# Findeton/mpi-vision

Hardware: AMD Instinct MI355X
Metric: rendered Mpix/sec (node) + achieved HBM GB/s fraction, 1024²×128-plane MPI (higher is better)
Workload: dtype f32

## Files before the change

### mpi_vision_amd/csrc/abi.hip

```cpp
#include <cstdio>
#include <cstdarg>
#include <cstring>
#include <cstdlib>
#include <algorithm>
#include <mutex>
#include <type_traits>

#include "../../include/mpiv.h"

#ifndef MPIV_AB
#define MPIV_AB 0
#endif
#include "render.hip"
#include "render_lds.hip"
#include "render_chunk.hip"
#include "render_ring.hip"
#include "render_mv.hip"
#include "render_bwd.hip"
#include "render_bwd_cam.hip"
#include "sweep.hip"
#include "warp_bwd.hip"
#include "psv_bwd.hip"
#include "helper_bwd.hip"
#include "geometry.hip"
#include "assemble.hip"
#include "synth.hip"
#include "render_texel.hip"

namespace {

thread_local char g_err[512] = "";

int fail(int code, const char* fmt, ...) {
    va_list ap;
    va_start(ap, fmt);
    vsnprintf(g_err, sizeof(g_err), fmt, ap);
    va_end(ap);
    return code;
}

int launched(const char* what) {
    const hipError_t e = hipGetLastError();
    if (e != hipSuccess) return fail(MPIV_ERR_HIP, "%s: launch failed: %s", what, hipGetErrorString(e));
    g_err[0] = '\0';
    return MPIV_OK;
}

inline hipStream_t S(void* s) { return reinterpret_cast<hipStream_t>(s); }
inline bool aligned16(const void* p) { return (reinterpret_cast<uintptr_t>(p) & 15) == 0; }
inline unsigned blocks(int64_t n, int per) { return (unsigned)((n + per - 1) / per); }

enum DebugOpt { kOptRenderMv, kOptRenderPair, kOptNativeLds, kOptSweepTile, kOptSweepStore, kOptBoxShrink,
                kOptRenderChunk, kOptRenderRing, kOptRenderTile, kOptBwdFallback, kOptBwdMargin, kOptSweepDlane,
                kOptRenderVshare, kOptChunkRows, kOptSweepRows, kOptChunkFlight, kOptBwdGather, kOptSweepDirect,
                kOptBwdPollLimit, kOptBwdFbBlocks, kOptBwdFbMode, kOptChunkStrip, kOptU8Flight, kOptBwdGroup,
                kOptNetoutGeo, kOptNetoutBuf, kOptBwdOverlap, kOptSweepBand, kOptSweepPf, kOptSweepSoa, kOptBwdUnfold,
                kOptNetoutFg3, kOptRenderSame, kOptRenderColsep, kOptRenderOrder, kOptChunkWide, kNumOpts };
const char* const kOptNames[kNumOpts] = {"render_mv", "render_pair", "render_native_lds",
                                         "sweep_tile", "sweep_store", "box_shrink", "render_chunk", "render_ring",
                                         "render_tile", "bwd_fallback", "bwd_margin", "sweep_dlane",
                                         "render_vshare", "chunk_rows", "sweep_rows", "chunk_flight", "bwd_gather",
                                         "sweep_direct", "bwd_poll_limit", "bwd_fb_blocks", "bwd_fb_mode",
                                         "chunk_strip", "u8_flight", "bwd_group", "netout_geo", "netout_buf", "bwd_overlap", "sweep_band",
                                         "sweep_pf", "sweep_soa", "bwd_unfold", "netout_fg3",
                                         "render_same", "render_colsep", "render_order", "chunk_wide"};
#ifndef MPIV_CHUNK_STRIP
#define MPIV_CHUNK_STRIP 1
#endif
#ifndef MPIV_U8_FLIGHT
#define MPIV_U8_FLIGHT 0
#endif
const int kOptDefaults[kNumOpts] = {0, 0, 1, 0, -1, 0, 0, 0, 0, 0, 16, 1, 0, 0, 0, 0, 0, 0, 0, 0, 0, MPIV_CHUNK_STRIP,
                                    MPIV_U8_FLIGHT, 0, 0, 1, 0, 0, 0, 0, 0, 1, 0, 0, 0, 0};
int g_opts[kNumOpts] = {0, 0, 1, 0, -1, 0, 0, 0, 0, 0, 16, 1, 0, 0, 0, 0, 0, 0, 0, 0, 0, MPIV_CHUNK_STRIP, MPIV_U8_FLIGHT, 0,
                        0, 1, 0, 0, 0, 0, 0, 1, 0, 0, 0, 0};

int opt(DebugOpt o) { return __atomic_load_n(&g_opts[o], __ATOMIC_RELAXED); }

bool ab_only(int o, int v) {
    switch (o) {
        case kOptRenderMv: case kOptRenderPair: case kOptSweepTile: return v != 0;
        case kOptRenderRing: return v > 0;
        case kOptRenderTile: return v != 0 && v != -1;
        case kOptRenderVshare: return v == -1 || v == 1;
        case kOptSweepStore: return v >= 0;
        case kOptRenderChunk: return v >= 100;
        case kOptSweepDlane: return v == 0;
        case kOptChunkRows: return v == 2 || v == 4;
        case kOptChunkFlight: return v == 4;
        case kOptChunkStrip: return v >= 2;
        case kOptSweepRows: return v == 6 || v == 8;
        case kOptBwdGather: return v == 1 || v == 2 || v == 3;
        case kOptBwdPollLimit: case kOptBwdFbBlocks: case kOptBwdFbMode: return v != 0;
        case kOptBwdOverlap: case kOptSweepBand: return v != 0;
        case kOptSweepPf: case kOptSweepSoa: return v > 0;
        default: return false;
    }
}

thread_local unsigned long long* g_census = nullptr;

struct RouteNote {
    char name[160];
    int64_t threads;
};
thread_local RouteNote* g_route = nullptr;

int note_route(int64_t blocks_, int threads, const char* fmt, ...) {
    va_list ap;
    va_start(ap, fmt);
    vsnprintf(g_route->name, sizeof(g_route->name), fmt, ap);
    va_end(ap);
    g_route->threads = blocks_ * threads;
    return MPIV_OK;
}

constexpr int64_t kMaxGridYZ = 65535;
constexpr int kNativeLdsMaxP = 16;
constexpr int kChunkMaxLds = 65536;
constexpr int kChunkSplit = 1;

constexpr int64_t kMaxGridX = 2147483647;

constexpr const char* kViewTooLarge = "%s: one view is limited to H*W < 2^26 and P*H*W < 2^31 (32 GiB of fp32 RGBA)";
inline bool view_too_large(int H, int W, int P) {
    return (int64_t)H * W >= ((int64_t)1 << 26) || (int64_t)P * H * W >= ((int64_t)1 << 31);
}

}

using namespace mpiv;

namespace {

constexpr int kOrderMinViews = 64;
int render_tile_order(int V) {
    const int o = opt(kOptRenderOrder);
    return o > 0 ? 1 : o < 0 ? 0 : V >= kOrderMinViews ? 1 : 0;
}

int chunk_rows() {
    const int o = opt(kOptChunkRows);
    return (o == 2 || o == 4) ? o : 1;
}

template <int CH, int SPLIT>
int launch_chunk(int R, const float* mpi, int64_t vstride, const RenderGeom& g, const ChunkGeom& cg, int B,
                 const float* homs, float* out, float4* ck, size_t lds, hipStream_t q, const char* nm,
                 bool wide = false) {
    if constexpr (CH == 8 && SPLIT == 1) {
        if (wide) {
            const int64_t ns = (int64_t)blocks(g.W, kStripTX) * blocks(g.H, 16) * B;
            if (ns > kMaxGridX) return fail(MPIV_ERR_ARG, "%s: too many blocks", nm);
            if (g_route) return note_route(ns, 256, "render_chunk_strip_kernel<16, 2, true>");
            render_chunk_strip_kernel<16, 2, true><<<(unsigned)ns, 256, lds, q>>>(mpi, vstride, g, cg, B, homs, out, ck);
            return launched(nm);
        }
    }
    const int64_t nb = (int64_t)blocks(g.W, kTileX) * blocks(g.H, kTileY * R) * B;
    if (nb > kMaxGridX) return fail(MPIV_ERR_ARG, "%s: too many blocks", nm);
    const int NT = (opt(kOptChunkFlight) == 4 && R == 1 && SPLIT == 1) ? 4 : 2;
    const int so = opt(kOptChunkStrip);
    if (CH == 8 && SPLIT == 1 && R == 1 && NT == 2 && so > 0) {
        const int SR = (so == 2 || so == 3) ? 8 : 16, SNT = so >= 3 ? 3 : 2;
        const int64_t ns = (int64_t)blocks(g.W, kStripTX) * blocks(g.H, SR) * B;
        if (ns > kMaxGridX) return fail(MPIV_ERR_ARG, "%s: too many blocks", nm);
        if (g_route) return note_route(ns, 256, "render_chunk_strip_kernel<%d, %d>", SR, SNT);
#if MPIV_AB
        if (so == 2)
            render_chunk_strip_kernel<8, 2><<<(unsigned)ns, 256, lds, q>>>(mpi, vstride, g, cg, B, homs, out, ck);
        else if (so == 3)
            render_chunk_strip_kernel<8, 3><<<(unsigned)ns, 256, lds, q>>>(mpi, vstride, g, cg, B, homs, out, ck);
        else if (so == 4)
// ... 261 lines not shown
    const int rows_opt = opt(kOptRenderTile);
    const int64_t rows_blocks = (int64_t)blocks(W, kTileX) * blocks(H, 4 * 8) * V;
    const bool stretched_vs = !square && rows_blocks >= 2048;
    const bool variants_off = !opt(kOptRenderMv) && !opt(kOptRenderPair);
    const int rows_auto = ((square || stretched_vs) && variants_off) ? 8 : 0;
    const int vs_opt = opt(kOptRenderVshare);
    [[maybe_unused]] const int rows_sel = fast ? (rows_opt ? rows_opt : rows_auto) : 0;
#if MPIV_AB
    if (const int rows = rows_sel; rows == 108 || rows == 116 || rows == 132) {
        const int R = rows - 100;
        const int64_t nb = (int64_t)blocks(W, kTileX) * blocks(H, 4 * R) * V;
        if (nb > kMaxGridX) return fail(MPIV_ERR_ARG, "%s: too many blocks", nm);
#define MPIV_ROWSL(R)                                                                                                  \
    if (ct)                                                                                                           \
        render_rows_lds_kernel<true, R><<<(unsigned)nb, 256, 0, st>>>(pk, ps, g, V, p_begin, p_end, back, homs, out); \
    else                                                                                                              \
        render_rows_lds_kernel<false, R><<<(unsigned)nb, 256, 0, st>>>(pk, ps, g, V, p_begin, p_end, 1, homs, out)
        if (R == 8) MPIV_ROWSL(8);
        else if (R == 16) MPIV_ROWSL(16);
        else MPIV_ROWSL(32);
#undef MPIV_ROWSL
        return launched(nm);
    }
#endif

    int vsd = 0;
    if (fast && (vs_opt == 3 || vs_opt == 4 || vs_opt == 5 || vs_opt == 11))
        vsd = vs_opt;
    else if (fast && vs_opt == 0 && !rows_opt && rows_auto == 8)
        vsd = rows_same(syr) ? 4 : V <= 2 ? 11 : V <= 8 ? 3 : square ? 4 : 5;
    if (vsd) {
        const int R = vsd == 3 ? 8 : vsd == 4 ? 6 : vsd == 5 ? 9 : 4;
        const int64_t nb = (int64_t)blocks(W, kTileX) * blocks(H, 4 * R) * V;
        if (nb > kMaxGridX) return fail(MPIV_ERR_ARG, "%s: too many blocks", nm);
        const bool same = rows_same(syr);
        const bool oob = same && vsd == 4 && rows_same_oob(V);
        if (g_route)
            return note_route(nb, 256, "render_rows_%s<%s, %d, true, false, %d, %s, %s>", tgt ? "tgt_kernel" : "kernel",
                              ct ? "true" : "false", R, vsd == 3 || vsd == 11 ? 4 : 3, same ? "true" : "false",
                              oob ? "true" : "false");
        unsigned long long* cn = (g_census && !ct) ? g_census : nullptr;
        if (cn) g_census = nullptr;
        const int csp = opt(kOptRenderColsep);
        const int ord = render_tile_order(V);
#define MPIV_VSD(R, D, SM, OB)                                                                                        \
    if (ct)                                                                                                          \
        render_rows_kernel<true, R, true, false, D, SM, OB><<<(unsigned)nb, 256, 0, st>>>(                           \
            pk, ps, g, V, p_begin, p_end, back, homs, out, nullptr, 0, -1, csp, ord);                                \
    else if (tgt)                                                                                                    \
        render_rows_tgt_kernel<false, R, true, false, D, SM, OB><<<(unsigned)nb, 256, 0, st>>>(                      \
            pk, ps, gt, V, p_begin, p_end, 1, homs, out, nullptr, 0, -1, csp, ord);                                  \
    else                                                                                                             \
        render_rows_kernel<false, R, true, false, D, SM, OB><<<(unsigned)nb, 256, 0, st>>>(                          \
            pk, ps, g, V, p_begin, p_end, 1, homs, out, nullptr, 0, -1, csp, ord)
#define MPIV_VSDC(R, D, SM, OB)                                                                                       \
    if (cn)                                                                                                          \
        render_rows_kernel<false, R, true, true, D, SM, OB><<<(unsigned)nb, 256, 0, st>>>(                           \
            pk, ps, g, V, p_begin, p_end, 1, homs, out, cn, 0, -1, csp, ord);                                        \
    else                                                                                                             \
        MPIV_VSD(R, D, SM, OB)
        if (oob) {
            MPIV_VSDC(6, 3, true, true);
        } else if (same) {
            switch (vsd) {
                case 3: MPIV_VSDC(8, 4, true, false); break;
                case 4: MPIV_VSDC(6, 3, true, false); break;
                case 5: MPIV_VSDC(9, 3, true, false); break;
                default: MPIV_VSDC(4, 4, true, false); break;
            }
        } else {
            switch (vsd) {
                case 3: MPIV_VSDC(8, 4, false, false); break;
                case 4: MPIV_VSDC(6, 3, false, false); break;
                case 5: MPIV_VSDC(9, 3, false, false); break;
                default: MPIV_VSDC(4, 4, false, false); break;
            }
        }
#undef MPIV_VSDC
#undef MPIV_VSD
        return launched(nm);
    }
#if MPIV_AB
    if (const int rows = rows_sel; rows == 2 || rows == 4 || rows == 8 || rows == 16) {
        const int64_t nb = (int64_t)blocks(W, kTileX) * blocks(H, 4 * rows) * V;
        if (nb > kMaxGridX) return fail(MPIV_ERR_ARG, "%s: too many blocks", nm);
#define MPIV_ROWS(R)                                                                                               \
    if (ct)                                                                                                       \
        render_rows_kernel<true, R><<<(unsigned)nb, 256, 0, st>>>(pk, ps, g, V, p_begin, p_end, back, homs, out); \
    else                                                                                                          \
// ... 72 lines not shown
int mpiv_render_packed_lds(const float* packed, int H, int W, int P, const float* homs, int V, float* out,
                           void* stream) {
#if !MPIV_AB
    (void)packed, (void)H, (void)W, (void)P, (void)homs, (void)V, (void)out, (void)stream;
    return fail(MPIV_ERR_ARG, "mpiv_render_packed_lds: an A/B kernel, built only into libmpiv_ab.so");
#endif
    return render_packed_impl(packed, H, W, H, W, P, 0, P, 1, homs, V, out, false, 1, stream);
}

int mpiv_render_packed_ct(const float* packed, int H, int W, int P, int p_begin, int p_end, int back,
                          const float* homs, int V, float* ct, void* stream) {
    return render_packed_impl(packed, H, W, H, W, P, p_begin, p_end, back, homs, V, ct, true, 0, stream);
}

int mpiv_render_packed_ct_rows(const float* packed, int H, int W, int P, int p_begin, int p_end, int back,
                               const float* homs, int V, int y_begin, int y_end, float* ct, void* stream) {
    const char* nm = "mpiv_render_packed_ct_rows";
    if (!packed || !homs || !ct) return fail(MPIV_ERR_ARG, "%s: null pointer", nm);
    if (V <= 0 || H < 2 || W < 2 || P <= 0) return fail(MPIV_ERR_ARG, "%s: bad shape (H, W >= 2)", nm);
    if (p_begin < 0 || p_end > P || p_begin >= p_end) return fail(MPIV_ERR_ARG, "%s: bad plane range", nm);
    if (y_begin < 0 || y_end > H || y_begin >= y_end) return fail(MPIV_ERR_ARG, "%s: bad row range", nm);
    if (!aligned16(packed) || !aligned16(ct)) return fail(MPIV_ERR_ARG, "%s: 16-byte alignment", nm);
    if ((int64_t)(H + 2 * kPad) * (W + 2 * kPad) * 16 >= (int64_t)kOOB || H >= (1 << 22) || W >= (1 << 22))
        return fail(MPIV_ERR_ARG, "%s: padded plane larger than 2 GiB or a side >= 2^22", nm);
    const float4* pk = reinterpret_cast<const float4*>(packed);
    const int64_t ps = (int64_t)(H + 2 * kPad) * (W + 2 * kPad);
    const RenderGeom g = make_geom(H, W, P);
    const float sxr = (float)W / (float)(H - 1), syr = (float)H / (float)(W - 1);
    const bool square = sxr >= 0.8f && sxr <= 1.25f && syr >= 0.8f && syr <= 1.25f;
    const bool same = rows_same(syr);
    const bool oob = same && rows_same_oob(V);
    const int R = same ? 6 : V <= 2 ? 4 : V <= 8 ? 8 : square ? 6 : 9;
    const int64_t nb = (int64_t)blocks(W, kTileX) * blocks(y_end - y_begin, 4 * R) * V;
    if (nb > kMaxGridX) return fail(MPIV_ERR_ARG, "%s: too many blocks", nm);
    if (g_route)
        return note_route(nb, 256, "render_rows_kernel<true, %d, true, false, %d, %s, %s>", R, R == 4 || R == 8 ? 4 : 3,
                          same ? "true" : "false", oob ? "true" : "false");
    hipStream_t st = S(stream);
    const int csp = opt(kOptRenderColsep);
    const int ord = render_tile_order(V);
#define MPIV_CTR(RR, DD, SM)                                                                                           \
    render_rows_kernel<true, RR, true, false, DD, SM><<<(unsigned)nb, 256, 0, st>>>(pk, ps, g, V, p_begin, p_end, back, \
                                                                                    homs, ct, nullptr, y_begin, y_end, csp, ord)
    if (oob) {
        render_rows_kernel<true, 6, true, false, 3, true, true><<<(unsigned)nb, 256, 0, st>>>(
            pk, ps, g, V, p_begin, p_end, back, homs, ct, nullptr, y_begin, y_end, csp, ord);
    } else if (same) {
        switch (R) {
            case 4: MPIV_CTR(4, 4, true); break;
            case 8: MPIV_CTR(8, 4, true); break;
            case 6: MPIV_CTR(6, 3, true); break;
            default: MPIV_CTR(9, 3, true); break;
        }
    } else {
        switch (R) {
            case 4: MPIV_CTR(4, 4, false); break;
            case 8: MPIV_CTR(8, 4, false); break;
            case 6: MPIV_CTR(6, 3, false); break;
            default: MPIV_CTR(9, 3, false); break;
        }
    }
#undef MPIV_CTR
    return launched(nm);
}


namespace {

inline size_t align256(size_t n) { return (n + 255) & ~(size_t)255; }

int bwd_group_planes(int H, int W, int P) {
    const int64_t n = (int64_t)P * H * W, cap = (int64_t)1 << 25;
    if (H < 2 || W < 2) return P;
    if (opt(kOptBwdGroup) > 0) return std::min(P, (opt(kOptBwdGroup) + kBwdCH - 1) / kBwdCH * kBwdCH);
    if (n <= cap) return P;
    const int64_t groups = (n + cap - 1) / cap;
    const int gp = (int)(((int64_t)P + groups - 1) / groups);
    return std::min(P, (gp + kBwdCH - 1) / kBwdCH * kBwdCH);
}

size_t bwd_layout(int H, int W, int P, int dsp, char* base, BwdWs* ws, float4** gbuf = nullptr, int nwin = 1,
                  BwdWs* ws2 = nullptr) {
    const size_t hw = (size_t)H * W;
    const int pc = bwd_group_planes(H, W, P);
    const size_t nk = (size_t)pc * (H + 1) * (W + 1);
    const size_t nb = (nk + kScanTile - 1) / kScanTile;
    const size_t nchunk = (size_t)(P + kBwdCH - 1) / kBwdCH;
    size_t off = 0;
    auto take = [&](size_t bytes) {
        char* p = base ? base + off : nullptr;
        off += align256(bytes);
        return p;
    };
    char* truth = take(kCtrSlots * 8);
    char* found = take(kCtrSlots * 8);
// ... 1756 lines not shown
    if (!out) return fail(MPIV_ERR_ARG, "mpiv_tile_order: null pointer");
    if (ntiles <= 0 || tiles_x <= 0 || ntiles % tiles_x)
        return fail(MPIV_ERR_ARG, "mpiv_tile_order: bad shape (whole tile rows: ntiles a multiple of tiles_x)");
    if (order != -1 && order != 1) return fail(MPIV_ERR_ARG, "mpiv_tile_order: order must be -1 (band) or 1 (interleaved)");
    for (int t = 0; t < ntiles; ++t) out[t] = xcd_tile_order(t, ntiles, tiles_x, order);
    return MPIV_OK;
}

int mpiv_mark(int tag, void* stream) {
    if (tag < 1 || tag > 4096) return fail(MPIV_ERR_ARG, "mpiv_mark: tag must be in 1..4096");
    mark_kernel<<<tag, 64, 0, S(stream)>>>();
    return launched("mpiv_mark");
}

int mpiv_probe_gather(const float* window, size_t window_bytes, int iters, int blocks_, float* sink, void* stream) {
    if (!window || !sink) return fail(MPIV_ERR_ARG, "mpiv_probe_gather: null pointer");
    if (window_bytes < (size_t)kProbeWindow)
        return fail(MPIV_ERR_ARG, "mpiv_probe_gather: the window must hold >= %d bytes", (int)kProbeWindow);
    if (iters <= 0 || blocks_ <= 0) return fail(MPIV_ERR_ARG, "mpiv_probe_gather: bad size");
    if (!aligned16(window)) return fail(MPIV_ERR_ARG, "mpiv_probe_gather: window must be 16-byte aligned");
    probe_gather_kernel<<<blocks_, 256, 0, S(stream)>>>(reinterpret_cast<const float4*>(window), iters, sink);
    return launched("mpiv_probe_gather");
}

int mpiv_route(const char* entry, const int64_t* a, int na, char* name, int name_cap, int64_t* grid_threads) {
    if (!entry || !a || !name || name_cap <= 0) return fail(MPIV_ERR_ARG, "mpiv_route: null pointer");
    for (int i = 0; i < kNumOpts; ++i)
        if (opt((DebugOpt)i) != kOptDefaults[i])
            return fail(MPIV_ERR_ARG, "mpiv_route: reports the production routes only (debug options are set)");
    alignas(256) static float dummy[64];
    float* d = dummy;
    RouteNote note{};
    int rc;
    g_route = &note;
    if (strcmp(entry, "render_packed") == 0 && na == 4)
        rc = render_packed_impl(d, (int)a[0], (int)a[1], (int)a[0], (int)a[1], (int)a[2], 0, (int)a[2], 1, d, (int)a[3], d, false, 0,
                                nullptr);
    else if (strcmp(entry, "render_packed_ct") == 0 && na == 4)
        rc = render_packed_impl(d, (int)a[0], (int)a[1], (int)a[0], (int)a[1], (int)a[2], 0, (int)a[2], 1, d, (int)a[3], d, true, 0,
                                nullptr);
    else if (strcmp(entry, "render_packed_ct_rows") == 0 && na == 6)
        rc = mpiv_render_packed_ct_rows(d, (int)a[0], (int)a[1], (int)a[2], 0, (int)a[2], 1, d, (int)a[3], (int)a[4],
                                        (int)a[5], d, nullptr);
    else if (strcmp(entry, "plane_sweep") == 0 && na == 7) {
        const int64_t C = a[3], D = a[4], st[4] = {a[1] * a[2] * C, a[2] * C, C, 1};
        rc = mpiv_plane_sweep(d, st, (int)a[0], (int)a[1], (int)a[2], (int)C, d, d, d, (int)D, (int)a[5], (int)a[6], d,
                              nullptr);
    } else if (strcmp(entry, "render_train") == 0 && na == 4) {
        const int64_t P = a[3], st[5] = {a[1] * a[2] * P * 4, a[2] * P * 4, P * 4, 4, 1};
        rc = mpiv_render_train(d, st, (int)a[0], (int)a[1], (int)a[2], (int)P, d, d, d, nullptr);
    } else if (strcmp(entry, "render_backward") == 0 && na == 4) {
        const int64_t P = a[3], st[5] = {a[1] * a[2] * P * 4, a[2] * P * 4, P * 4, 4, 1};
        const float* ck = a[1] >= 2 && a[2] >= 2 ? d : nullptr;
        rc = mpiv_render_backward(d, st, (int)a[0], (int)a[1], (int)a[2], (int)P, d, d, ck, d, d,
                                  mpiv_render_backward_workspace_size((int)a[1], (int)a[2], (int)P), nullptr);
    } else if (strcmp(entry, "render_packed_u8") == 0 && na == 4) {
        rc = render_tex_impl<TexU8>(d, (int)a[0], (int)a[1], (int)a[0], (int)a[1], (int)a[2], 0, (int)a[2], 1, d, (int)a[3], d,
                                    false, nullptr);
    } else if ((strcmp(entry, "render_packed_f16") == 0 || strcmp(entry, "render_packed_f16_ct") == 0) && na == 4) {
        rc = render_tex_impl<TexF16>(d, (int)a[0], (int)a[1], (int)a[0], (int)a[1], (int)a[2], 0, (int)a[2], 1, d, (int)a[3], d,
                                     strcmp(entry, "render_packed_f16_ct") == 0, nullptr);
    } else if (strcmp(entry, "render_packed_tgt") == 0 && na == 6) {
        rc = render_packed_impl(d, (int)a[0], (int)a[1], (int)a[4], (int)a[5], (int)a[2], 0, (int)a[2], 1, d, (int)a[3], d,
                                false, 0, nullptr, "mpiv_render_packed_tgt");
    } else if (strcmp(entry, "render_packed_u8_tgt") == 0 && na == 6) {
        rc = render_tex_impl<TexU8>(d, (int)a[0], (int)a[1], (int)a[4], (int)a[5], (int)a[2], 0, (int)a[2], 1, d, (int)a[3], d,
                                    false, nullptr, "mpiv_render_packed_u8_tgt");
    } else if (strcmp(entry, "render_packed_f16_tgt") == 0 && na == 6) {
        rc = render_tex_impl<TexF16>(d, (int)a[0], (int)a[1], (int)a[4], (int)a[5], (int)a[2], 0, (int)a[2], 1, d, (int)a[3], d,
                                     false, nullptr, "mpiv_render_packed_f16_tgt");
    } else if (strcmp(entry, "render_packed_alpha") == 0 && na == 4) {
        rc = mpiv_render_packed_alpha(d, (int)a[0], (int)a[1], (int)a[2], d, d, (int)a[3], d, nullptr);
    } else if (strcmp(entry, "render_net_output") == 0 && na == 4) {
        const int64_t B = a[0], H = a[1], W = a[2], P = a[3];
        const int64_t ps[4] = {(2 * P + 3) * H * W, H * W, W, 1}, fs[4] = {H * W * 3, W * 3, 3, 1};
        rc = mpiv_render_net_output(d, ps, d, fs, (int)B, (int)H, (int)W, (int)P, d, d, nullptr);
    } else if (strcmp(entry, "render") == 0 && na == 4) {
        const int64_t P = a[3], st[5] = {a[1] * a[2] * P * 4, a[2] * P * 4, P * 4, 4, 1};
        rc = mpiv_render(d, st, (int)a[0], (int)a[1], (int)a[2], (int)P, d, d, nullptr);
    } else {
        g_route = nullptr;
        return fail(MPIV_ERR_ARG, "mpiv_route: unknown entry '%s' or wrong argument count %d", entry, na);
    }
    g_route = nullptr;
    if (rc != MPIV_OK) return rc;
    if (!note.name[0]) return fail(MPIV_ERR_ARG, "mpiv_route: '%s' has no reportable route", entry);
    snprintf(name, (size_t)name_cap, "%s", note.name);
    if (grid_threads) *grid_threads = note.threads;
    g_err[0] = '\0';
    return MPIV_OK;
}

int mpiv_selftest_tickets(int blocks_, int nphase, int nvirt, unsigned poll_limit, unsigned* ctr, int* marks,
                          void* stream) {
#if MPIV_AB
    if (!ctr || !marks || blocks_ <= 0 || nphase <= 0 || nvirt <= 0) return fail(MPIV_ERR_ARG, "mpiv_selftest_tickets: bad args");
    ticket_selftest_kernel<<<blocks_, 256, 0, S(stream)>>>(ctr, marks, nphase, nvirt, poll_limit);
    return launched("mpiv_selftest_tickets");
#else
    (void)blocks_, (void)nphase, (void)nvirt, (void)poll_limit, (void)ctr, (void)marks, (void)stream;
    return fail(MPIV_ERR_ARG, "mpiv_selftest_tickets: an A/B diagnosis, built only into libmpiv_ab.so");
#endif
}

int mpiv_selftest_div_const(int divisor, unsigned long long* mismatches, void* stream) {
    if (!mismatches || divisor < 1) return fail(MPIV_ERR_ARG, "mpiv_selftest_div_const: bad args");
    const float c = (float)divisor;
    div_const_selftest_kernel<<<4096, 256, 0, S(stream)>>>(c, 1.0f / c, mismatches);
    return launched("mpiv_selftest_div_const");
}

}
```

### mpi_vision_amd/csrc/render.hip

```cpp
#include "mpiv_common.hpp"

namespace mpiv {

constexpr int kTileX = 64;
constexpr int kTileY = 4;

struct RenderGeom {
    int H, W, P;
    int Wp;
    int org;
    int row;
    int plane_bytes;
    float hm1, wm1;
    float rc_hm1, rc_wm1;
    float half_w, half_h;
};

inline RenderGeom make_geom(int H, int W, int P) {
    RenderGeom g;
    g.H = H; g.W = W; g.P = P;
    g.Wp = W + 2 * kPad;
    g.row = g.Wp * 16;
    g.org = (kPad * g.Wp + kPad) * 16;
    g.plane_bytes = (int)((int64_t)(H + 2 * kPad) * g.Wp * 16);
// ... 169 lines not shown
}

template <bool CT>
__device__ __forceinline__ void composite_zero(int p_begin, int p_end, bool replace_first, float& cr, float& cg,
                                               float& cb, float& t) {
    for (int p = p_begin; p < p_end; ++p) {
        const float a = (replace_first && p == p_begin) ? 1.0f : 0.0f;
        const float om = 1.0f - a;
        cr = over(0.0f, a, om, cr);
        cg = over(0.0f, a, om, cg);
        cb = over(0.0f, a, om, cb);
        if (CT) t = t * om;
    }
}


__device__ __forceinline__ int xcd_logical_block(int b, int nblocks) {
    const int q = nblocks >> 3, r = nblocks & 7;
    const int xcd = b & 7, k = b >> 3;
    return xcd * q + (xcd < r ? xcd : r) + k;
}

__host__ __device__ __forceinline__ int xcd_tile_order(int t, int ntiles, int tiles_x, int order) {
    if (order <= 0) return t;
    const int q = ntiles >> 3, r = ntiles & 7;
    const int x = t < r * (q + 1) ? t / (q + 1) : r + (t - r * (q + 1)) / (q > 1 ? q : 1);
    const int k = t - (x * q + (x < r ? x : r));
    const int e = k * 8 + x;
    const int ty = e / tiles_x;
    const int g = (tiles_x | 8) & -(tiles_x | 8);
    const int rot = (int)(((int64_t)ty * g) >> 3);
    const int tx = (e % tiles_x + tiles_x - rot % tiles_x) % tiles_x;
    return ty * tiles_x + tx;
}

template <bool CT, int MODE>
__device__ __forceinline__ void render_packed_pixel(const float4* __restrict__ planes, int64_t plane_stride,
                                                    const RenderGeom& g, int p_begin, int p_end, int back,
                                                    const float* __restrict__ hv, int x, int y,
                                                    float* __restrict__ out_px) {
    const float fx = (float)x, fy = (float)y;
    float cr = -0.0f, cg = -0.0f, cb = -0.0f, t = 1.0f;
    const bool replace_first = !CT || back;
    const int last = p_end - 1;
    auto hom = [&](int p) { return load_hom(hv + (int64_t)(p < last ? p : last) * 9); };
    auto issue = [&](int p, const Hom9& h, TapSet& ts) {
        const int q = p < last ? p : last;
        float px, py;
        if (MODE == 0)
            render_pos<false>(h.h, fx, fy, g, px, py);
        else
            render_pos_fast<MODE == 1>(h.h, fx, fy, g, px, py);
        issue_taps_padded(make_rsrc(planes + (int64_t)q * plane_stride, g.plane_bytes), g.W, g.H, g.Wp, g.org,
                          g.row, px, py, ts);
    };
    auto consume = [&](const TapSet& ts, bool first) {
        const f32x4 s = blend_taps(ts);
        const float a = first ? 1.0f : s[3];
        const float om = 1.0f - a;
        cr = over(s[0], a, om, cr);
        cg = over(s[1], a, om, cg);
        cb = over(s[2], a, om, cb);
        if (CT) t = t * om;
    };
    TapSet A, B;
    Hom9 hA = hom(p_begin), hB = hom(p_begin + 1);
// ... 681 lines not shown
```

### mpi_vision_amd/csrc/render_kernels.inc

```

template <bool CT, bool FAST>
__global__ __launch_bounds__(256) void MPIV_KERNEL(render_packed)(const float4* __restrict__ planes,
                                                            int64_t plane_stride, MPIV_GEOM g, int V,
                                                            int p_begin, int p_end, int back,
                                                            const float* __restrict__ homs,
                                                            float* __restrict__ out, int order = 0) {
    const int tiles_x = (tgt_w(g) + kTileX - 1) / kTileX;
    const int lb = xcd_logical_block(blockIdx.x, gridDim.x);
    const int v = lb % V;
    const int tile = xcd_tile_order(lb / V, (int)gridDim.x / V, tiles_x, order);
    const int tx0 = (tile % tiles_x) * kTileX, ty0 = (tile / tiles_x) * kTileY;
    const int x = tx0 + (threadIdx.x & (kWave - 1));
    const int y = ty0 + (threadIdx.x >> 6);
    const float* hv = homs + (int64_t)v * g.P * 9;
    bool proven = false, dead = false;
    if (FAST) {
        const float x0 = (float)tx0, x1 = (float)min(tx0 + kTileX - 1, tgt_w(g) - 1);
        const float y0 = (float)ty0, y1 = (float)min(ty0 + kTileY - 1, tgt_h(g) - 1);
        bool ok = true, dd = true;
        for (int p = p_begin + (int)threadIdx.x; p < p_end; p += 256) {
            const float* hp = hv + (int64_t)p * 9;
            const bool safe = div2_rect_safe(hp, x0, x1, y0, y1);
            ok = ok && safe;
            dd = dd && safe && tile_dead(hp, x0, x1, y0, y1, g);
        }
        proven = __syncthreads_and(ok);
        dead = __syncthreads_and(dd);
    }
    if (x >= tgt_w(g) || y >= tgt_h(g)) return;
    const int64_t o = ((int64_t)v * tgt_h(g) + y) * tgt_w(g) + x;
    float* out_px = CT ? out + o * 4 : out + o * 3;
    if (dead) {
        float cr = -0.0f, cg = -0.0f, cb = -0.0f, t = 1.0f;
        composite_zero<CT>(p_begin, p_end, !CT || back, cr, cg, cb, t);
        if (CT) {
            *reinterpret_cast<float4*>(out_px) = make_float4(cr, cg, cb, t);
        } else {
            out_px[0] = cr;
            out_px[1] = cg;
            out_px[2] = cb;
        }
        return;
    }
    if (!FAST)
        render_packed_pixel<CT, 0>(planes, plane_stride, g, p_begin, p_end, back, hv, x, y, out_px);
    else if (proven)
        render_packed_pixel<CT, 2>(planes, plane_stride, g, p_begin, p_end, back, hv, x, y, out_px);
    else
        render_packed_pixel<CT, 1>(planes, plane_stride, g, p_begin, p_end, back, hv, x, y, out_px);
}

template <bool CT, int R, bool VS = false, bool COUNT = false, int D = 2, bool SAME = false, bool OOB = false>
__global__ __launch_bounds__(256) __attribute__((amdgpu_waves_per_eu(SAME && R == 6 && !OOB ? 4 : 1))) void MPIV_KERNEL(render_rows)(const float4* __restrict__ planes, int64_t plane_stride,
                                                          MPIV_GEOM g, int V, int p_begin, int p_end, int back,
                                                          const float* __restrict__ homs, float* __restrict__ out,
                                                          unsigned long long* __restrict__ census = nullptr,
                                                          int y_lo = 0, int y_hi = -1, int colsep = 0,
                                                          int order = 0) {
    constexpr int TY = 4 * R;
    if (y_hi < 0) y_hi = tgt_h(g);
    const int tiles_x = (tgt_w(g) + kTileX - 1) / kTileX;
    const int lb = xcd_logical_block(blockIdx.x, gridDim.x);
    const int v = lb % V;
    const int tile = xcd_tile_order(lb / V, (int)gridDim.x / V, tiles_x, order);
    const int tx0 = (tile % tiles_x) * kTileX, ty0 = y_lo + (tile / tiles_x) * TY;
    const int x = tx0 + (int)(threadIdx.x & (kWave - 1));
    const int y0 = ty0 + (int)(threadIdx.x >> 6) * R;
    const float* hv = homs + (int64_t)v * g.P * 9;
    bool ok = true, dd = true, cs = true;
    {
        const float x0 = (float)tx0, x1 = (float)min(tx0 + kTileX - 1, tgt_w(g) - 1);
        const float fy0 = (float)ty0, fy1 = (float)min(ty0 + TY - 1, tgt_h(g) - 1);
        for (int p = p_begin + (int)threadIdx.x; p < p_end; p += 256) {
            const float* hp = hv + (int64_t)p * 9;
            const bool safe = div2_rect_safe(hp, x0, x1, fy0, fy1);
            ok = ok && safe;
            dd = dd && safe && tile_dead(hp, x0, x1, fy0, fy1, g);
            cs = cs && hp[1] == 0.0f && hp[7] == 0.0f;
        }
    }
    const bool proven = __syncthreads_and(ok);
    const bool dead = __syncthreads_and(dd);
    constexpr bool COLSEP = VS && !(CT && SAME && R == 8);
    bool sep = false;
    if constexpr (COLSEP)
        sep = g.row < kColsepMaxPitch && (colsep > 0 || (colsep == 0 && __syncthreads_and(cs)));
    if (x >= tgt_w(g) || y0 >= y_hi) return;
    float cr[R], cg[R], cb[R], tt[R];
#pragma unroll
    for (int k = 0; k < R; ++k) {
        cr[k] = -0.0f; cg[k] = -0.0f; cb[k] = -0.0f; tt[k] = 1.0f;
    }
    if (dead) {
        composite_zero<CT>(p_begin, p_end, !CT || back, cr[0], cg[0], cb[0], tt[0]);
#pragma unroll
        for (int k = 1; k < R; ++k) {
            cr[k] = cr[0]; cg[k] = cg[0]; cb[k] = cb[0]; tt[k] = tt[0];
        }
    } else if (!proven) {
        int rows = 0;
        for (int k = 0; k < R && y0 + k < y_hi; ++k, ++rows) {
            const int64_t o = ((int64_t)v * tgt_h(g) + y0 + k) * tgt_w(g) + x;
            render_packed_pixel<CT, 1>(planes, plane_stride, g, p_begin, p_end, back, hv, x, y0 + k,
                                       CT ? out + o * 4 : out + o * 3);
        }
        if (COUNT && (threadIdx.x & (kWave - 1)) == 0)
            atomicAdd(census, (unsigned long long)rows * 4ull * (unsigned long long)(p_end - p_begin + 1));
        return;
    }
    auto store = [&]() {
#pragma unroll
        for (int k = 0; k < R; ++k) {
            const int y = y0 + k;
            if (y >= y_hi) break;
            const int64_t o = ((int64_t)v * tgt_h(g) + y) * tgt_w(g) + x;
            if (CT) {
                reinterpret_cast<float4*>(out)[o] = make_float4(cr[k], cg[k], cb[k], tt[k]);
            } else {
                out[o * 3 + 0] = cr[k];
                out[o * 3 + 1] = cg[k];
                out[o * 3 + 2] = cb[k];
            }
        }
    };
    if (!dead) {
        unsigned nvm = 0;
        if constexpr (VS) {
            if (COLSEP && sep) {
                render_rows_vs_pixels<CT, false, R, D, SAME, OOB, COLSEP>(planes, plane_stride, g, p_begin, p_end, back, hv,
                                                                        x, y0, cr, cg, cb, tt, nvm);
                if (COUNT && (threadIdx.x & (kWave - 1)) == 0) atomicAdd(census, (unsigned long long)nvm);
                store();
                return;
            }
            render_rows_vs_pixels<CT, false, R, D, SAME, OOB>(planes, plane_stride, g, p_begin, p_end, back, hv, x, y0, cr,
                                                              cg, cb, tt, nvm);
        } else
            render_rows_pixels<CT, false, R>(planes, plane_stride, g, p_begin, p_end, back, hv, x, y0, cr, cg, cb, tt);
        if (!VS) nvm = 4u * (unsigned)(R * (p_end - p_begin) + 1);
        if (COUNT && (threadIdx.x & (kWave - 1)) == 0) atomicAdd(census, (unsigned long long)nvm);
    }
    store();
}
```

Before: 5814.

## Add view-grouped row render kernel mapping waves to different views per block

Adds a render_rows_vg kernel variant in which each of the four waves in a block handles a strip for a different view rather than four row strips of one view. Tile-safety checks become per-wave ballots instead of block-wide syncthreads. It is enabled by default when V is at least 32. The aim is to group views that sample the same MPI region so they share cache, and to cut block-level syncs. In exchange, each wave checks the plane homographies on its own, so per-wave safety-check work grows, and the block mapping logic gets more complex.

Result: faster. 6051, median of 6 (+4.1%).

```diff
diff --git a/mpi_vision_amd/csrc/abi.hip b/mpi_vision_amd/csrc/abi.hip
--- a/mpi_vision_amd/csrc/abi.hip
+++ b/mpi_vision_amd/csrc/abi.hip
@@ -55,7 +55,8 @@
                 kOptRenderVshare, kOptChunkRows, kOptSweepRows, kOptChunkFlight, kOptBwdGather, kOptSweepDirect,
                 kOptBwdPollLimit, kOptBwdFbBlocks, kOptBwdFbMode, kOptChunkStrip, kOptU8Flight, kOptBwdGroup,
                 kOptNetoutGeo, kOptNetoutBuf, kOptBwdOverlap, kOptSweepBand, kOptSweepPf, kOptSweepSoa, kOptBwdUnfold,
-                kOptNetoutFg3, kOptRenderSame, kOptRenderColsep, kOptRenderOrder, kOptChunkWide, kNumOpts };
+                kOptNetoutFg3, kOptRenderSame, kOptRenderColsep, kOptRenderOrder, kOptChunkWide, kOptRenderVgroup,
+                kNumOpts };
 const char* const kOptNames[kNumOpts] = {"render_mv", "render_pair", "render_native_lds",
                                          "sweep_tile", "sweep_store", "box_shrink", "render_chunk", "render_ring",
                                          "render_tile", "bwd_fallback", "bwd_margin", "sweep_dlane",
@@ -63,7 +64,7 @@
                                          "sweep_direct", "bwd_poll_limit", "bwd_fb_blocks", "bwd_fb_mode",
                                          "chunk_strip", "u8_flight", "bwd_group", "netout_geo", "netout_buf", "bwd_overlap", "sweep_band",
                                          "sweep_pf", "sweep_soa", "bwd_unfold", "netout_fg3",
-                                         "render_same", "render_colsep", "render_order", "chunk_wide"};
+                                         "render_same", "render_colsep", "render_order", "chunk_wide", "render_vgroup"};
 #ifndef MPIV_CHUNK_STRIP
 #define MPIV_CHUNK_STRIP 1
 #endif
@@ -71,9 +72,9 @@
 #define MPIV_U8_FLIGHT 0
 #endif
 const int kOptDefaults[kNumOpts] = {0, 0, 1, 0, -1, 0, 0, 0, 0, 0, 16, 1, 0, 0, 0, 0, 0, 0, 0, 0, 0, MPIV_CHUNK_STRIP,
-                                    MPIV_U8_FLIGHT, 0, 0, 1, 0, 0, 0, 0, 0, 1, 0, 0, 0, 0};
+                                    MPIV_U8_FLIGHT, 0, 0, 1, 0, 0, 0, 0, 0, 1, 0, 0, 0, 0, 0};
 int g_opts[kNumOpts] = {0, 0, 1, 0, -1, 0, 0, 0, 0, 0, 16, 1, 0, 0, 0, 0, 0, 0, 0, 0, 0, MPIV_CHUNK_STRIP, MPIV_U8_FLIGHT, 0,
-                        0, 1, 0, 0, 0, 0, 0, 1, 0, 0, 0, 0};
+                        0, 1, 0, 0, 0, 0, 0, 1, 0, 0, 0, 0, 0};
 
 int opt(DebugOpt o) { return __atomic_load_n(&g_opts[o], __ATOMIC_RELAXED); }
 
@@ -105,6 +106,7 @@
     int64_t threads;
 };
 thread_local RouteNote* g_route = nullptr;
+thread_local bool g_route_launched = false;
 
 int note_route(int64_t blocks_, int threads, const char* fmt, ...) {
     va_list ap;
@@ -139,6 +141,12 @@
     return o > 0 ? 1 : o < 0 ? 0 : V >= kOrderMinViews ? 1 : 0;
 }
 
+constexpr int kVgroupMinViews = 32;
+int render_view_group(int V, int64_t nblocks) {
+    const int o = opt(kOptRenderVgroup);
+    if (V >= (1 << 28) || nblocks / V >= (1 << 28)) return 0;
+    return o > 0 ? 1 : o < 0 ? 0 : V >= kVgroupMinViews ? 1 : 0;
+}
 int chunk_rows() {
     const int o = opt(kOptChunkRows);
     return (o == 2 || o == 4) ? o : 1;
@@ -466,11 +474,13 @@
     if (vsd) {
         const int R = vsd == 3 ? 8 : vsd == 4 ? 6 : vsd == 5 ? 9 : 4;
         const int64_t nb = (int64_t)blocks(W, kTileX) * blocks(H, 4 * R) * V;
+        const int vg = tgt ? 0 : render_view_group(V, nb);
         if (nb > kMaxGridX) return fail(MPIV_ERR_ARG, "%s: too many blocks", nm);
         const bool same = rows_same(syr);
         const bool oob = same && vsd == 4 && rows_same_oob(V);
         if (g_route)
-            return note_route(nb, 256, "render_rows_%s<%s, %d, true, false, %d, %s, %s>", tgt ? "tgt_kernel" : "kernel",
+            return note_route(nb, 256, "render_rows_%s<%s, %d, true, false, %d, %s, %s>",
+                              tgt ? "tgt_kernel" : vg && g_route_launched ? "vg_kernel" : "kernel",
                               ct ? "true" : "false", R, vsd == 3 || vsd == 11 ? 4 : 3, same ? "true" : "false",
                               oob ? "true" : "false");
         unsigned long long* cn = (g_census && !ct) ? g_census : nullptr;
@@ -478,17 +488,26 @@
         const int csp = opt(kOptRenderColsep);
         const int ord = render_tile_order(V);
 #define MPIV_VSD(R, D, SM, OB)                                                                                        \
-    if (ct)                                                                                                          \
+    if (ct && vg)                                                                                                    \
+        render_rows_vg_kernel<true, R, true, false, D, SM, OB><<<(unsigned)nb, 256, 0, st>>>(                        \
+            pk, ps, g, V, p_begin, p_end, back, homs, out, nullptr, 0, -1, csp, ord);                                \
+    else if (ct)                                                                                                     \
         render_rows_kernel<true, R, true, false, D, SM, OB><<<(unsigned)nb, 256, 0, st>>>(                           \
             pk, ps, g, V, p_begin, p_end, back, homs, out, nullptr, 0, -1, csp, ord);                                \
     else if (tgt)                                                                                                    \
         render_rows_tgt_kernel<false, R, true, false, D, SM, OB><<<(unsigned)nb, 256, 0, st>>>(                      \
             pk, ps, gt, V, p_begin, p_end, 1, homs, out, nullptr, 0, -1, csp, ord);                                  \
+    else if (vg)                                                                                                     \
+        render_rows_vg_kernel<false, R, true, false, D, SM, OB><<<(unsigned)nb, 256, 0, st>>>(                       \
+            pk, ps, g, V, p_begin, p_end, 1, homs, out, nullptr, 0, -1, csp, ord);                                   \
     else                                                                                                             \
         render_rows_kernel<false, R, true, false, D, SM, OB><<<(unsigned)nb, 256, 0, st>>>(                          \
             pk, ps, g, V, p_begin, p_end, 1, homs, out, nullptr, 0, -1, csp, ord)
 #define MPIV_VSDC(R, D, SM, OB)                                                                                       \
-    if (cn)                                                                                                          \
+    if (cn && vg)                                                                                                    \
+        render_rows_vg_kernel<false, R, true, true, D, SM, OB><<<(unsigned)nb, 256, 0, st>>>(                        \
+            pk, ps, g, V, p_begin, p_end, 1, homs, out, cn, 0, -1, csp, ord);                                        \
+    else if (cn)                                                                                                     \
         render_rows_kernel<false, R, true, true, D, SM, OB><<<(unsigned)nb, 256, 0, st>>>(                           \
             pk, ps, g, V, p_begin, p_end, 1, homs, out, cn, 0, -1, csp, ord);                                        \
     else                                                                                                             \
@@ -627,19 +646,24 @@
     const bool oob = same && rows_same_oob(V);
     const int R = same ? 6 : V <= 2 ? 4 : V <= 8 ? 8 : square ? 6 : 9;
     const int64_t nb = (int64_t)blocks(W, kTileX) * blocks(y_end - y_begin, 4 * R) * V;
+    const int vg = render_view_group(V, nb);
     if (nb > kMaxGridX) return fail(MPIV_ERR_ARG, "%s: too many blocks", nm);
     if (g_route)
-        return note_route(nb, 256, "render_rows_kernel<true, %d, true, false, %d, %s, %s>", R, R == 4 || R == 8 ? 4 : 3,
+        return note_route(nb, 256, "render_rows_%s<true, %d, true, false, %d, %s, %s>",
+                          vg && g_route_launched ? "vg_kernel" : "kernel", R, R == 4 || R == 8 ? 4 : 3,
                           same ? "true" : "false", oob ? "true" : "false");
     hipStream_t st = S(stream);
     const int csp = opt(kOptRenderColsep);
     const int ord = render_tile_order(V);
-#define MPIV_CTR(RR, DD, SM)                                                                                           \
-    render_rows_kernel<true, RR, true, false, DD, SM><<<(unsigned)nb, 256, 0, st>>>(pk, ps, g, V, p_begin, p_end, back, \
-                                                                                    homs, ct, nullptr, y_begin, y_end, csp, ord)
+#define MPIV_CTRV(KERNEL, RR, DD, SM, OB)                                                    \
+    KERNEL<true, RR, true, false, DD, SM, OB><<<(unsigned)nb, 256, 0, st>>>(                 \
+        pk, ps, g, V, p_begin, p_end, back, homs, ct, nullptr, y_begin, y_end, csp, ord)
+#define MPIV_CTR(RR, DD, SM)                                        \
+    if (vg) MPIV_CTRV(render_rows_vg_kernel, RR, DD, SM, false); \
+    else MPIV_CTRV(render_rows_kernel, RR, DD, SM, false)
     if (oob) {
-        render_rows_kernel<true, 6, true, false, 3, true, true><<<(unsigned)nb, 256, 0, st>>>(
-            pk, ps, g, V, p_begin, p_end, back, homs, ct, nullptr, y_begin, y_end, csp, ord);
+        if (vg) MPIV_CTRV(render_rows_vg_kernel, 6, 3, true, true);
+        else MPIV_CTRV(render_rows_kernel, 6, 3, true, true);
     } else if (same) {
         switch (R) {
             case 4: MPIV_CTR(4, 4, true); break;
@@ -656,6 +680,7 @@
         }
     }
 #undef MPIV_CTR
+#undef MPIV_CTRV
     return launched(nm);
 }
 
@@ -2478,6 +2503,27 @@
     float* d = dummy;
     RouteNote note{};
     int rc;
+    if (strcmp(entry, "view_group_pair") == 0 && na == 6) {
+        const int64_t nt = a[0], tx = a[1], V = a[3];
+        if (nt <= 0 || tx <= 0 || nt % tx || (a[2] != -1 && a[2] != 1) || V <= 0 || V >= (1 << 28) || nt >= (1 << 28) ||
+            nt * V > kMaxGridX || a[4] < 0 || a[4] >= nt * V || a[5] < 0 || a[5] > 3)
+            return fail(MPIV_ERR_ARG, "mpiv_route: view_group_pair: bad arguments");
+        int v, strip;
+        view_group_pair((int)a[4], (int)a[5], (int)nt, (int)V, (int)tx, (int)a[2], v, strip);
+        snprintf(name, (size_t)name_cap, "view %d, strip %d", v, strip);
+        if (grid_threads) *grid_threads = (int64_t)strip * V + v;
+        g_err[0] = '\0';
+        return MPIV_OK;
+    }
+    char base[64];
+    if (const char* colon = strchr(entry, ':')) {
+        if (strcmp(colon, ":launched") != 0 || (size_t)(colon - entry) >= sizeof(base))
+            return fail(MPIV_ERR_ARG, "mpiv_route: unknown entry '%s'", entry);
+        memcpy(base, entry, (size_t)(colon - entry));
+        base[colon - entry] = '\0';
+        entry = base;
+        g_route_launched = true;
+    }
     g_route = &note;
     if (strcmp(entry, "render_packed") == 0 && na == 4)
         rc = render_packed_impl(d, (int)a[0], (int)a[1], (int)a[0], (int)a[1], (int)a[2], 0, (int)a[2], 1, d, (int)a[3], d, false, 0,
@@ -2526,9 +2572,11 @@
         rc = mpiv_render(d, st, (int)a[0], (int)a[1], (int)a[2], (int)P, d, d, nullptr);
     } else {
         g_route = nullptr;
+        g_route_launched = false;
         return fail(MPIV_ERR_ARG, "mpiv_route: unknown entry '%s' or wrong argument count %d", entry, na);
     }
     g_route = nullptr;
+    g_route_launched = false;
     if (rc != MPIV_OK) return rc;
     if (!note.name[0]) return fail(MPIV_ERR_ARG, "mpiv_route: '%s' has no reportable route", entry);
     snprintf(name, (size_t)name_cap, "%s", note.name);
diff --git a/mpi_vision_amd/csrc/render.hip b/mpi_vision_amd/csrc/render.hip
--- a/mpi_vision_amd/csrc/render.hip
+++ b/mpi_vision_amd/csrc/render.hip
@@ -225,6 +225,13 @@
     const int rot = (int)(((int64_t)ty * g) >> 3);
     const int tx = (e % tiles_x + tiles_x - rot % tiles_x) % tiles_x;
     return ty * tiles_x + tx;
+}
+
+__host__ __device__ __forceinline__ void view_group_pair(int lb, int w, int ntiles, int V, int tiles_x, int order,
+                                                         int& v, int& strip) {
+    const int q = lb / V, kr = (lb % V) * 4 + w;
+    v = kr % V;
+    strip = xcd_tile_order(q * 4 + kr / V, ntiles * 4, tiles_x, order);
 }
 
 template <bool CT, int MODE>
diff --git a/mpi_vision_amd/csrc/render_kernels.inc b/mpi_vision_amd/csrc/render_kernels.inc
--- a/mpi_vision_amd/csrc/render_kernels.inc
+++ b/mpi_vision_amd/csrc/render_kernels.inc
@@ -50,95 +50,13 @@
         render_packed_pixel<CT, 1>(planes, plane_stride, g, p_begin, p_end, back, hv, x, y, out_px);
 }
 
-template <bool CT, int R, bool VS = false, bool COUNT = false, int D = 2, bool SAME = false, bool OOB = false>
-__global__ __launch_bounds__(256) __attribute__((amdgpu_waves_per_eu(SAME && R == 6 && !OOB ? 4 : 1))) void MPIV_KERNEL(render_rows)(const float4* __restrict__ planes, int64_t plane_stride,
-                                                          MPIV_GEOM g, int V, int p_begin, int p_end, int back,
-                                                          const float* __restrict__ homs, float* __restrict__ out,
-                                                          unsigned long long* __restrict__ census = nullptr,
-                                                          int y_lo = 0, int y_hi = -1, int colsep = 0,
-                                                          int order = 0) {
-    constexpr int TY = 4 * R;
-    if (y_hi < 0) y_hi = tgt_h(g);
-    const int tiles_x = (tgt_w(g) + kTileX - 1) / kTileX;
-    const int lb = xcd_logical_block(blockIdx.x, gridDim.x);
-    const int v = lb % V;
-    const int tile = xcd_tile_order(lb / V, (int)gridDim.x / V, tiles_x, order);
-    const int tx0 = (tile % tiles_x) * kTileX, ty0 = y_lo + (tile / tiles_x) * TY;
-    const int x = tx0 + (int)(threadIdx.x & (kWave - 1));
-    const int y0 = ty0 + (int)(threadIdx.x >> 6) * R;
-    const float* hv = homs + (int64_t)v * g.P * 9;
-    bool ok = true, dd = true, cs = true;
-    {
-        const float x0 = (float)tx0, x1 = (float)min(tx0 + kTileX - 1, tgt_w(g) - 1);
-        const float fy0 = (float)ty0, fy1 = (float)min(ty0 + TY - 1, tgt_h(g) - 1);
-        for (int p = p_begin + (int)threadIdx.x; p < p_end; p += 256) {
-            const float* hp = hv + (int64_t)p * 9;
-            const bool safe = div2_rect_safe(hp, x0, x1, fy0, fy1);
-            ok = ok && safe;
-            dd = dd && safe && tile_dead(hp, x0, x1, fy0, fy1, g);
-            cs = cs && hp[1] == 0.0f && hp[7] == 0.0f;
-        }
-    }
-    const bool proven = __syncthreads_and(ok);
-    const bool dead = __syncthreads_and(dd);
-    constexpr bool COLSEP = VS && !(CT && SAME && R == 8);
-    bool sep = false;
-    if constexpr (COLSEP)
-        sep = g.row < kColsepMaxPitch && (colsep > 0 || (colsep == 0 && __syncthreads_and(cs)));
-    if (x >= tgt_w(g) || y0 >= y_hi) return;
-    float cr[R], cg[R], cb[R], tt[R];
-#pragma unroll
-    for (int k = 0; k < R; ++k) {
-        cr[k] = -0.0f; cg[k] = -0.0f; cb[k] = -0.0f; tt[k] = 1.0f;
-    }
-    if (dead) {
-        composite_zero<CT>(p_begin, p_end, !CT || back, cr[0], cg[0], cb[0], tt[0]);
-#pragma unroll
-        for (int k = 1; k < R; ++k) {
-            cr[k] = cr[0]; cg[k] = cg[0]; cb[k] = cb[0]; tt[k] = tt[0];
-        }
-    } else if (!proven) {
-        int rows = 0;
-        for (int k = 0; k < R && y0 + k < y_hi; ++k, ++rows) {
-            const int64_t o = ((int64_t)v * tgt_h(g) + y0 + k) * tgt_w(g) + x;
-            render_packed_pixel<CT, 1>(planes, plane_stride, g, p_begin, p_end, back, hv, x, y0 + k,
-                                       CT ? out + o * 4 : out + o * 3);
-        }
-        if (COUNT && (threadIdx.x & (kWave - 1)) == 0)
-            atomicAdd(census, (unsigned long long)rows * 4ull * (unsigned long long)(p_end - p_begin + 1));
-        return;
-    }
-    auto store = [&]() {
-#pragma unroll
-        for (int k = 0; k < R; ++k) {
-            const int y = y0 + k;
-            if (y >= y_hi) break;
-            const int64_t o = ((int64_t)v * tgt_h(g) + y) * tgt_w(g) + x;
-            if (CT) {
-                reinterpret_cast<float4*>(out)[o] = make_float4(cr[k], cg[k], cb[k], tt[k]);
-            } else {
-                out[o * 3 + 0] = cr[k];
-                out[o * 3 + 1] = cg[k];
-                out[o * 3 + 2] = cb[k];
-            }
-        }
-    };
-    if (!dead) {
-        unsigned nvm = 0;
-        if constexpr (VS) {
-            if (COLSEP && sep) {
-                render_rows_vs_pixels<CT, false, R, D, SAME, OOB, COLSEP>(planes, plane_stride, g, p_begin, p_end, back, hv,
-                                                                        x, y0, cr, cg, cb, tt, nvm);
-                if (COUNT && (threadIdx.x & (kWave - 1)) == 0) atomicAdd(census, (unsigned long long)nvm);
-                store();
-                return;
-            }
-            render_rows_vs_pixels<CT, false, R, D, SAME, OOB>(planes, plane_stride, g, p_begin, p_end, back, hv, x, y0, cr,
-                                                              cg, cb, tt, nvm);
-        } else
-            render_rows_pixels<CT, false, R>(planes, plane_stride, g, p_begin, p_end, back, hv, x, y0, cr, cg, cb, tt);
-        if (!VS) nvm = 4u * (unsigned)(R * (p_end - p_begin) + 1);
-        if (COUNT && (threadIdx.x & (kWave - 1)) == 0) atomicAdd(census, (unsigned long long)nvm);
-    }
-    store();
-}
+#define MPIV_VG 0
+#define MPIV_ROWS_KERNEL MPIV_KERNEL(render_rows)
+#include "render_rows.inc"
+#undef MPIV_ROWS_KERNEL
+#undef MPIV_VG
+#define MPIV_VG 1
+#define MPIV_ROWS_KERNEL MPIV_KERNEL(render_rows_vg)
+#include "render_rows.inc"
+#undef MPIV_ROWS_KERNEL
+#undef MPIV_VG
diff --git a/mpi_vision_amd/csrc/render_rows.inc b/mpi_vision_amd/csrc/render_rows.inc
--- /dev/null
+++ b/mpi_vision_amd/csrc/render_rows.inc
@@ -0,0 +1,104 @@
+template <bool CT, int R, bool VS = false, bool COUNT = false, int D = 2, bool SAME = false, bool OOB = false>
+__global__ __launch_bounds__(256) __attribute__((amdgpu_waves_per_eu(SAME && R == 6 && !OOB ? 4 : 1))) void MPIV_ROWS_KERNEL(const float4* __restrict__ planes, int64_t plane_stride,
+                                                          MPIV_GEOM g, int V, int p_begin, int p_end, int back,
+                                                          const float* __restrict__ homs, float* __restrict__ out,
+                                                          unsigned long long* __restrict__ census = nullptr,
+                                                          int y_lo = 0, int y_hi = -1, int colsep = 0,
+                                                          int order = 0) {
+    constexpr bool VG = MPIV_VG != 0;
+    constexpr int TY = 4 * R;
+    if (y_hi < 0) y_hi = tgt_h(g);
+    const int tiles_x = (tgt_w(g) + kTileX - 1) / kTileX;
+    const int lb = xcd_logical_block(blockIdx.x, gridDim.x);
+    int v, tx0, ty0, y0, th, first, stride;
+    if constexpr (VG) {
+        int strip;
+        view_group_pair(lb, __builtin_amdgcn_readfirstlane((int)(threadIdx.x >> 6)), (int)gridDim.x / V, V, tiles_x,
+                        order, v, strip);
+        tx0 = (strip % tiles_x) * kTileX, y0 = ty0 = y_lo + (strip / tiles_x) * R;
+        if (y0 >= y_hi) return;
+        th = R, first = (int)(threadIdx.x & (kWave - 1)), stride = kWave;
+    } else {
+        v = lb % V;
+        const int tile = xcd_tile_order(lb / V, (int)gridDim.x / V, tiles_x, order);
+        tx0 = (tile % tiles_x) * kTileX, ty0 = y_lo + (tile / tiles_x) * TY;
+        y0 = ty0 + (int)(threadIdx.x >> 6) * R;
+        th = TY, first = (int)threadIdx.x, stride = 256;
+    }
+    const int x = tx0 + (int)(threadIdx.x & (kWave - 1));
+    const float* hv = homs + (int64_t)v * g.P * 9;
+    bool ok = true, dd = true, cs = true;
+    {
+        const float x0 = (float)tx0, x1 = (float)min(tx0 + kTileX - 1, tgt_w(g) - 1);
+        const float fy0 = (float)ty0, fy1 = (float)min(ty0 + th - 1, tgt_h(g) - 1);
+        for (int p = p_begin + first; p < p_end; p += stride) {
+            const float* hp = hv + (int64_t)p * 9;
+            const bool safe = div2_rect_safe(hp, x0, x1, fy0, fy1);
+            ok = ok && safe;
+            dd = dd && safe && tile_dead(hp, x0, x1, fy0, fy1, g);
+            cs = cs && hp[1] == 0.0f && hp[7] == 0.0f;
+        }
+    }
+    const bool proven = VG ? __all(ok) : __syncthreads_and(ok);
+    const bool dead = VG ? __all(dd) : __syncthreads_and(dd);
+    constexpr bool COLSEP = VS && !(CT && SAME && R == 8);
+    bool sep = false;
+    if constexpr (COLSEP)
+        sep = g.row < kColsepMaxPitch && (colsep > 0 || (colsep == 0 && (VG ? __all(cs) : __syncthreads_and(cs))));
+    if (x >= tgt_w(g) || y0 >= y_hi) return;
+    float cr[R], cg[R], cb[R], tt[R];
+#pragma unroll
+    for (int k = 0; k < R; ++k) {
+        cr[k] = -0.0f; cg[k] = -0.0f; cb[k] = -0.0f; tt[k] = 1.0f;
+    }
+    if (dead) {
+        composite_zero<CT>(p_begin, p_end, !CT || back, cr[0], cg[0], cb[0], tt[0]);
+#pragma unroll
+        for (int k = 1; k < R; ++k) {
+            cr[k] = cr[0]; cg[k] = cg[0]; cb[k] = cb[0]; tt[k] = tt[0];
+        }
+    } else if (!proven) {
+        int rows = 0;
+        for (int k = 0; k < R && y0 + k < y_hi; ++k, ++rows) {
+            const int64_t o = ((int64_t)v * tgt_h(g) + y0 + k) * tgt_w(g) + x;
+            render_packed_pixel<CT, 1>(planes, plane_stride, g, p_begin, p_end, back, hv, x, y0 + k,
+                                       CT ? out + o * 4 : out + o * 3);
+        }
+        if (COUNT && (threadIdx.x & (kWave - 1)) == 0)
+            atomicAdd(census, (unsigned long long)rows * 4ull * (unsigned long long)(p_end - p_begin + 1));
+        return;
+    }
+    auto store = [&]() {
+#pragma unroll
+        for (int k = 0; k < R; ++k) {
+            const int y = y0 + k;
+            if (y >= y_hi) break;
+            const int64_t o = ((int64_t)v * tgt_h(g) + y) * tgt_w(g) + x;
+            if (CT) {
+                reinterpret_cast<float4*>(out)[o] = make_float4(cr[k], cg[k], cb[k], tt[k]);
+            } else {
+                out[o * 3 + 0] = cr[k];
+                out[o * 3 + 1] = cg[k];
+                out[o * 3 + 2] = cb[k];
+            }
+        }
+    };
+    if (!dead) {
+        unsigned nvm = 0;
+        if constexpr (VS) {
+            if (COLSEP && sep) {
+                render_rows_vs_pixels<CT, false, R, D, SAME, OOB, COLSEP>(planes, plane_stride, g, p_begin, p_end, back, hv,
+                                                                        x, y0, cr, cg, cb, tt, nvm);
+                if (COUNT && (threadIdx.x & (kWave - 1)) == 0) atomicAdd(census, (unsigned long long)nvm);
+                store();
+                return;
+            }
+            render_rows_vs_pixels<CT, false, R, D, SAME, OOB>(planes, plane_stride, g, p_begin, p_end, back, hv, x, y0, cr,
+                                                              cg, cb, tt, nvm);
+        } else
+            render_rows_pixels<CT, false, R>(planes, plane_stride, g, p_begin, p_end, back, hv, x, y0, cr, cg, cb, tt);
+        if (!VS) nvm = 4u * (unsigned)(R * (p_end - p_begin) + 1);
+        if (COUNT && (threadIdx.x & (kWave - 1)) == 0) atomicAdd(census, (unsigned long long)nvm);
+    }
+    store();
+}
```
